# NVIDIA-AI-IOT/redtail

Hardware: AMD Instinct MI355X
Metric: stereo pairs/sec, ResNet18-2D 1257x369 (higher is better)
Workload: dtype f32

## Files before the change

redtail_amd/csrc/kernels/conv_mfma.hip.h:

```cpp
#pragma once
#include <type_traits>
#include "common.hip.h"

namespace rt {

struct ZSlice {
    int pad_y, pad_x;
    int Ho, Wo;
    int ch_row;
    unsigned tap_mask;
    int64_t y_off;
    int64_t w_off;
    int64_t r_off;
    int64_t r_off_il8;
    int64_t y_off_il8;
    int64_t r_off_il4;
};

struct ConvArgs {
    const float* x;
    float* y;
    const float* w;
    const float* bias;
    const float* resid;
    unsigned long long* dbg;
    const float* zeros;
    const ZSlice* zs;
    const int* ch_off;
    int CinPad;
    int Cout;
    int Hi, Wi;
    int x_pitch;
    int Ho, Wo;
    int pad_y, pad_x;
    int nz;
    int tiles_x;
    int act;
    int xcd_order;
    int64_t x_bstride;
    int64_t y_bstride;
    int64_t y_cstride;
    int64_t y_zstride;
    int64_t y_off;
    int y_ystride, y_xstride;
    int64_t r_cstride;
    int64_t r_bstride;
    int r_il8;
    int batch;
    int cin_real;
    int64_t x_cstride;
    const int* ch_shift;
    int w_exact;
    int z_inner;
    int nb_inner;
    int dw_seg, dw_nseg, dw_cpc, dw_ntiles;
    const float* x2;
    int x2_from;
};

#define RT_WG_TILE_NB(p, tile, zi, n, nblk)                                                         \
    int tile = blockIdx.x;                                                                          \
    if ((p).xcd_order) {                           \
        const int nwg_ = gridDim.x, q_ = nwg_ >> 3, r_ = nwg_ & 7;                                  \
        const int xcd_ = blockIdx.x & 7, idx_ = blockIdx.x >> 3;                                    \
        tile = (xcd_ < r_ ? xcd_ * (q_ + 1) : r_ * (q_ + 1) + (xcd_ - r_) * q_) + idx_;             \
    }                                                                                               \
    int nblk = blockIdx.y;                                                                          \
    if ((p).nb_inner > 0) { nblk = tile % (p).nb_inner; tile /= (p).nb_inner; }                     \
    int zi, n;                                                                                      \
    if ((p).z_inner) { zi = tile % (p).nz; tile /= (p).nz; n = blockIdx.z; }                        \
    else { zi = blockIdx.z % (p).nz; n = blockIdx.z / (p).nz; }
#define RT_WG_TILE(p, tile, zi, n) RT_WG_TILE_NB(p, tile, zi, n, nblk_unused_); (void)nblk_unused_;

#ifdef RT_KERNEL_TIMING
#define RT_TSTAMP() do { if (dbgp && tid == 0 && dbi < 16) dbgp[dbi++] = __builtin_amdgcn_s_memtime(); } while (0)
#else
#define RT_TSTAMP() do { } while (0)
#endif

#ifndef RT_ABLATE
#define RT_ABLATE 0
#endif
constexpr bool kAblGather = (RT_ABLATE & 1) != 0;
constexpr bool kAblWLoad = (RT_ABLATE & 2) != 0;
constexpr bool kAblLdsWr = (RT_ABLATE & 4) != 0;
constexpr bool kAblBarrier = (RT_ABLATE & 8) != 0;
constexpr bool kAblResid = (RT_ABLATE & 16) != 0;
constexpr bool kAblStore = (RT_ABLATE & 32) != 0;
constexpr bool kAblLdsRd = (RT_ABLATE & 64) != 0;
constexpr bool kAblXform = (RT_ABLATE & 128) != 0;
constexpr bool kAblMfma = (RT_ABLATE & 256) != 0;
__device__ __forceinline__ void wg_barrier() { if (!kAblBarrier) __syncthreads(); }

template <int N> struct VecOf;
template <> struct VecOf<2> { typedef float type __attribute__((ext_vector_type(2))); };
template <> struct VecOf<4> { typedef float type __attribute__((ext_vector_type(4))); };

template <int KH, int KW, int S, int TY, int TXW, int NBW, int CC, int NW = 4, bool WLDS = true>
struct ConvCfg {
    static constexpr int TX = 32 * TXW;
    static constexpr int NB = 32 * NBW;
    static constexpr int TAPS = KH * KW;
    static constexpr int CPG = CC / 2;
    static constexpr int PR = (TY - 1) * S + KH;
    static constexpr int PC = (TX - 1) * S + KW;
// ... 384 lines not shown
```

redtail_amd/csrc/kernels/conv_split.hip.h:

```cpp
#pragma once
#include <type_traits>
#include "common.hip.h"
#include "conv_mfma.hip.h"

namespace rt {

constexpr float kSplitScale = 2048.f;
constexpr float kSplitInv = 1.f / 2048.f;

struct S3Split {
    f16x4 hi, lo;
};
__device__ static __forceinline__ S3Split s3_split(f32x4 v) {
    S3Split s;
#ifdef HIPEMU
#pragma unroll
    for (int j = 0; j < 4; j++) {
        const _Float16 h = (_Float16)v[j];
        s.hi[j] = h;
        s.lo[j] = (_Float16)((v[j] - (float)h) * kSplitScale);
    }
#else
    unsigned h[2], l[2];
#pragma unroll
// ... 156 lines not shown
#pragma unroll
        for (int r = 0; r < 16; r++) { acc_m[r] = 0.f; acc_c[r] = 0.f; }
        const char* xb = sX[buf] + b_off;
#pragma unroll
        for (int t = 0; t < 9; t++) {
            const int r = t / 3, s = t % 3;
#pragma unroll
            for (int c = 0; c < 2; c++) {
                const char* bp = xb + (r * PC + s) * PXB + c * 32;
                const f16x8 bh = *reinterpret_cast<const f16x8*>(bp);
                const f16x8 bl = *reinterpret_cast<const f16x8*>(bp + 64);
                const f16x8 ah = __builtin_bit_cast(f16x8, sW[a_off + ((t * 2 + c) * 2 + 0) * 64]);
                const f16x8 al = __builtin_bit_cast(f16x8, sW[a_off + ((t * 2 + c) * 2 + 1) * 64]);
                acc_m = __builtin_amdgcn_mfma_f32_32x32x16_f16(ah, bh, acc_m, 0, 0, 0);
                acc_c = __builtin_amdgcn_mfma_f32_32x32x16_f16(al, bh, acc_c, 0, 0, 0);
                acc_c = __builtin_amdgcn_mfma_f32_32x32x16_f16(ah, bl, acc_c, 0, 0, 0);
            }
        }

        RT_TSTAMP();
        const buf_rsrc rs_y = make_buf(elem_ptr(p.y, (int64_t)n * p.y_bstride + p.y_off, 4));
        auto epilogue = [&](auto ACT) {
#pragma unroll
            for (int q = 0; q < 4; q++) {
                f32x4 o;
#pragma unroll
                for (int e = 0; e < 4; e++)
                    o[e] = apply_act_fast(fmaf(acc_c[4 * q + e], kSplitInv, acc_m[4 * q + e]) + (bias4[q][e] + rr[q][e]), decltype(ACT)::value);
                if constexpr (YIL) {
                    const unsigned vo = (inb && 8 * q + 4 * kg < p.Cout) ? (unsigned)((oy * p.y_ystride + ox) * 4 + 4 * kg * cs32) * 4u : kBufOOB;
                    buf_store4(o, rs_y, vo, (unsigned)(8 * q * cs32) * 4u);
                } else {
                    const unsigned vo = inb ? (unsigned)(oy * p.y_ystride + ox * p.y_xstride + 4 * kg * cs32) * 4u : kBufOOB;
#pragma unroll
                    for (int e = 0; e < 4; e++)
                        buf_store(o[e], rs_y, (8 * q + 4 * kg + e < p.Cout) ? vo : kBufOOB, (unsigned)((8 * q + e) * cs32) * 4u);
                }
            }
        };
        if (act == 1) epilogue(std::integral_constant<int, 1>{});
        else if (act == 2) epilogue(std::integral_constant<int, 2>{});
        else epilogue(std::integral_constant<int, 0>{});
        RT_TSTAMP();
    }
#ifdef RT_KERNEL_TIMING
    __builtin_amdgcn_s_waitcnt(0);
    if (dbgp && tid == 0) { dbgp[14] = __builtin_amdgcn_s_memtime(); dbgp[15] = __builtin_amdgcn_s_memrealtime() - rt0; }
#endif
}

}

namespace rt {

template <int KH, int KW, int S, int NW_ = 4>
struct S3Cfg {
    static constexpr int NW = NW_, TY = NW_, TX = 32, CC = 16, TAPS = KH * KW, NT = 64 * NW_;
    static constexpr int PR = (TY - 1) * S + KH, PC = (TX - 1) * S + KW;
    static constexpr int PCH = (PC + 1) / 2;
    static constexpr int PCL = S == 2 ? 2 * PCH : PC;
    static constexpr int NPART = NW / 4;
    static constexpr int NPIX = PR * PC, NKP = ((NPIX + NPART - 1) / NPART + 63) / 64;
    static constexpr int PXB = 80;
    static constexpr int W_SLOTS = TAPS * 2 * 2 * 32;
    static constexpr int NK_W = (W_SLOTS + NT - 1) / NT;
    static constexpr int IN_BYTES = PR * PCL * PXB, GRP_BYTES = IN_BYTES + W_SLOTS * 16;
    static constexpr int KS_MAX = NW_ != 4 ? 1 : (S == 2 ? 2 : 4);
    static constexpr int max_groups(int want) {
        int ks = want < 1 ? 1 : (want > KS_MAX ? KS_MAX : want);
        while (ks > 1 && (ks == 3 || ks * GRP_BYTES < (ks - 1) * NW * 64 * 16 * 4)) ks--;
        return ks;
    }
    static_assert(IN_BYTES % 16 == 0, "weight image alignment");
    static_assert(S == 1 || S == 2, "stride 1 or 2");
};

#ifndef RT_S3_WAVES
#define RT_S3_WAVES(S) ((S) == 2 ? 2 : 4)
#endif
template <int KH, int KW, int S, bool XIL, bool YIL, int NW = 4, typename TIN = float, typename TOUT = float>
__global__ void __launch_bounds__(64 * NW * (S3Cfg<KH, KW, S, NW>::KS_MAX)) RT_WAVES_PER_EU(RT_S3_WAVES(S)) conv_s3_kernel(ConvArgs p) {
    using Cfg = S3Cfg<KH, KW, S, NW>;
    constexpr bool XF16 = std::is_same<TIN, _Float16>::value, YF16 = std::is_same<TOUT, _Float16>::value;
    constexpr unsigned ESX = Io<TIN>::ES, ESY = Io<TOUT>::ES;
    static_assert(!XIL || !XF16, "interleaved fp16 input: conv_f16mma_kernel");
    constexpr int TY = Cfg::TY, TX = Cfg::TX, CC = Cfg::CC, TAPS = Cfg::TAPS, PC = Cfg::PC, PCL = Cfg::PCL, PXB = Cfg::PXB;
    constexpr int NKP = Cfg::NKP, NK_W = Cfg::NK_W, NT = Cfg::NT;

    constexpr int IN_BYTES = Cfg::IN_BYTES, GRP_BYTES = Cfg::GRP_BYTES;
#ifdef HIPEMU
    HIP_DYNAMIC_SHARED(char, smem)
#else
    extern __shared__ __attribute__((aligned(16))) char smem[];
#endif

    const int tid_wg = threadIdx.x;
    const int KS = Cfg::KS_MAX == 1 ? 1 : __builtin_amdgcn_readfirstlane((int)blockDim.x / NT);
    const int kgi = Cfg::KS_MAX == 1 ? 0 : __builtin_amdgcn_readfirstlane(tid_wg / NT);
    const int tid = tid_wg - kgi * NT;
    char* const sIn = smem + kgi * GRP_BYTES;
    f32x4* const sW = reinterpret_cast<f32x4*>(smem + kgi * GRP_BYTES + IN_BYTES);
#ifdef RT_KERNEL_TIMING
    unsigned long long* dbgp = (p.dbg && kgi == 0) ? p.dbg + ((size_t)(blockIdx.z * gridDim.y + blockIdx.y) * gridDim.x + blockIdx.x) * 16 : nullptr;
    int dbi = 0;
    const unsigned long long rt0 = __builtin_amdgcn_s_memrealtime();
#endif
// ... 4 lines not shown

    RT_WG_TILE_NB(p, tile, zi, n, nblk)
    const int tx0 = (tile % p.tiles_x) * TX;
    const int ty0 = (tile / p.tiles_x) * TY;
    const char* __restrict__ xb = elem_ptr(p.x, (int64_t)n * p.x_bstride, ESX);
    const int nchunks = p.CinPad / CC;
    int pad_y = p.pad_y, pad_x = p.pad_x, Ho = p.Ho, Wo = p.Wo, ch_row = zi;
    int64_t y_off = p.y_off + (int64_t)zi * p.y_zstride, w_off = 0, r_off = y_off, r_off_il8 = y_off;
    int64_t y_off_il4 = 4 * p.y_off + (int64_t)zi * p.y_zstride, r_off_il4 = y_off_il4;
    unsigned tap_mask = ~0u;
    if (p.zs) {
        const ZSlice z = p.zs[zi];
        pad_y = z.pad_y; pad_x = z.pad_x; Ho = z.Ho; Wo = z.Wo; ch_row = z.ch_row; y_off = z.y_off; w_off = z.w_off;
        r_off = z.r_off; r_off_il8 = z.r_off_il8;
        y_off_il4 = 4 * z.y_off;
        r_off_il4 = z.r_off_il4;
        tap_mask = z.tap_mask;
    }
    const int act = p.act;

    const int sg = wv & 3, spart = wv >> 2;
    const int* __restrict__ tab = p.ch_off + (int64_t)ch_row * p.CinPad + 4 * sg;
    unsigned voff[NKP];
    int lidx[NKP], xcol[NKP];
    const int* __restrict__ shtab = p.ch_shift ? p.ch_shift + (int64_t)ch_row * p.CinPad + 4 * sg : nullptr;
#pragma unroll
    for (int k = 0; k < NKP; k++) {
        const int pidx = spart * (NKP * 64) + lane + 64 * k;
        const int pr = pidx / PC, pc = pidx - pr * PC;
        const int iy = ty0 * S - pad_y + pr, ix = tx0 * S - pad_x + pc;
        const bool own = pidx < Cfg::NPIX && lane + 64 * k < NKP * 64;
        xcol[k] = ix;
        voff[k] = (own && iy >= 0 && iy < p.Hi && ix >= 0 && ix < p.Wi) ? (unsigned)(iy * p.x_pitch + ix) * (XIL ? 16u : ESX) : kBufOOB;
        const int col = S == 2 ? (pc & 1) * Cfg::PCH + (pc >> 1) : pc;
        lidx[k] = own ? (pr * PCL + col) * PXB + sg * 8 : -1;
    }
    const char* __restrict__ wsrc = reinterpret_cast<const char*>(p.w) + (w_off + ((int64_t)nblk * nchunks) * Cfg::W_SLOTS) * 16;
    const buf_rsrc rs_w = make_buf(wsrc);

    f32x4 rin[NKP];
    f32x4 rw[NK_W];
    auto prefetch = [&](int ch) {
        if constexpr (XIL) {
            const int off = tab[ch * CC];
            const int sh = shtab ? shtab[ch * CC] : 0;
            const buf_rsrc rs = make_buf(xb, off >= 0);
#pragma unroll
            for (int k = 0; k < NKP; k++) {
                const unsigned vo = sh == 0 ? voff[k] : ((voff[k] != kBufOOB && xcol[k] >= sh) ? voff[k] - (unsigned)sh * 16u : kBufOOB);
                rin[k] = buf_load4(rs, vo, (unsigned)off * 4u);
            }
        } else {
            const int sh = shtab ? shtab[ch * CC] : 0;
#pragma unroll
            for (int j = 0; j < 4; j++) {
                const int off = tab[ch * CC + j];
                const buf_rsrc rs = make_buf(xb, off >= 0);
#pragma unroll
                for (int k = 0; k < NKP; k++) {
                    const unsigned vo = sh == 0 ? voff[k] : ((voff[k] != kBufOOB && xcol[k] >= sh) ? voff[k] - (unsigned)sh * ESX : kBufOOB);
                    rin[k][j] = Io<TIN>::load(rs, vo, (unsigned)off * ESX);
                }
            }
        }
        const unsigned so = (unsigned)ch * (unsigned)(Cfg::W_SLOTS * 16);
#pragma unroll
        for (int k = 0; k < NK_W; k++) {
            const int idx = tid + NT * k;
            rw[k] = buf_load4(rs_w, idx < Cfg::W_SLOTS ? (unsigned)idx * 16u : kBufOOB, so);
        }
    };
    auto stage_to_lds = [&]() {
#pragma unroll
        for (int k = 0; k < NKP; k++) {
            if (lidx[k] < 0) continue;
            if constexpr (XF16) {
                f16x4 h;
#pragma unroll
                for (int j = 0; j < 4; j++) h[j] = (_Float16)rin[k][j];
                *reinterpret_cast<f16x4*>(sIn + lidx[k]) = h;
            } else {
                const S3Split s = s3_split(rin[k]);
                *reinterpret_cast<f16x4*>(sIn + lidx[k]) = s.hi;
                *reinterpret_cast<f16x4*>(sIn + lidx[k] + 32) = s.lo;
            }
        }
#pragma unroll
        for (int k = 0; k < NK_W; k++) {
            const int idx = tid + NT * k;
            if (idx < Cfg::W_SLOTS) sW[idx] = rw[k];
        }
    };

    const int64_t ybase = (int64_t)n * p.y_bstride + y_off;
    const int64_t rbase = (int64_t)n * p.r_bstride + r_off;
    const int cs32 = (int)p.y_cstride, rs32 = (int)p.r_cstride;
    const int oy = ty0 + wv, ox = tx0 + l31;
    const bool inb = oy < Ho && ox < Wo;
    const bool r_il = p.r_il8 != 0;
    const int cb = nblk * 32;
    f32x4 rr[4];
    if (p.resid != nullptr && kgi == 0) {
        const buf_rsrc rs_r = make_buf(elem_ptr(p.resid, r_il ? (int64_t)n * p.r_bstride + (YF16 ? r_off_il8 : r_off_il4) : rbase, ESY));
        if (r_il && YF16) {
            const unsigned vo = inb ? (unsigned)((oy * p.y_ystride + ox * p.y_xstride) * 8 + 4 * kg) * 2u : kBufOOB;
#pragma unroll
            for (int q = 0; q < 4; q++) {
                const u32x2_t u = __builtin_amdgcn_raw_buffer_load_b64(rs_r, (cb + 8 * q + 4 * kg < p.Cout) ? vo : kBufOOB, (unsigned)((cb + 8 * q) * rs32) * 2u, 0);
#pragma unroll
                for (int e = 0; e < 4; e++) rr[q][e] = (float)__builtin_bit_cast(_Float16, (unsigned short)(u[e >> 1] >> (16 * (e & 1))));
            }
        } else if (r_il) {
            const unsigned vo = inb ? (unsigned)((oy * p.y_ystride + ox * p.y_xstride) * 4 + 4 * kg * rs32) * 4u : kBufOOB;
#pragma unroll
            for (int q = 0; q < 4; q++) rr[q] = buf_load4(rs_r, (cb + 8 * q + 4 * kg < p.Cout) ? vo : kBufOOB, (unsigned)((cb + 8 * q) * rs32) * 4u);
        } else {
            const unsigned vo = inb ? (unsigned)(oy * p.y_ystride + ox * p.y_xstride + 4 * kg * rs32) * ESY : kBufOOB;
#pragma unroll
            for (int q = 0; q < 4; q++)
#pragma unroll
                for (int e = 0; e < 4; e++)
                    rr[q][e] = Io<TOUT>::load(rs_r, (cb + 8 * q + 4 * kg + e < p.Cout) ? vo : kBufOOB, (unsigned)((cb + 8 * q + e) * rs32) * ESY);
        }
    } else {
#pragma unroll
        for (int q = 0; q < 4; q++) rr[q] = f32x4{0.f, 0.f, 0.f, 0.f};
    }

    f32x16 acc_m, acc_c;
#pragma unroll
    for (int r = 0; r < 16; r++) { acc_m[r] = 0.f; acc_c[r] = 0.f; }
    const int a_off = kg * 32 + l31;
    const bool w_exact = p.w_exact != 0;
    const int b_off = (wv * S * PCL + l31) * PXB + kg * 16;
    auto compute = [&]() {
#pragma unroll
        for (int t = 0; t < TAPS; t++) {
            if (!((tap_mask >> t) & 1u)) continue;
            const int r = t / KW, s = t % KW;
            const int col = S == 2 ? (s & 1) * Cfg::PCH + (s >> 1) : s;
            const char* bp = sIn + b_off + (r * PCL + col) * PXB;
            const f16x8 bh = *reinterpret_cast<const f16x8*>(bp);
            const f16x8 ah = __builtin_bit_cast(f16x8, sW[a_off + (t * 2 + 0) * 64]);
            acc_m = __builtin_amdgcn_mfma_f32_32x32x16_f16(ah, bh, acc_m, 0, 0, 0);
            if (!w_exact) {
                const f16x8 al = __builtin_bit_cast(f16x8, sW[a_off + (t * 2 + 1) * 64]);
                acc_c = __builtin_amdgcn_mfma_f32_32x32x16_f16(al, bh, acc_c, 0, 0, 0);
            }
            if constexpr (!XF16) {
                const f16x8 bl = *reinterpret_cast<const f16x8*>(bp + 32);
                acc_c = __builtin_amdgcn_mfma_f32_32x32x16_f16(ah, bl, acc_c, 0, 0, 0);
            }
        }
    };

    if (kgi < nchunks) prefetch(kgi);
    RT_TSTAMP();
    for (int ch = kgi; ch < nchunks + kgi; ch += KS) {
        const bool mine = KS == 1 || ch < nchunks;
        if (ch != kgi) __syncthreads();
        if (mine) stage_to_lds();
        __syncthreads();
        RT_TSTAMP();
        if (ch + KS < nchunks) prefetch(ch + KS);
        if (mine) compute();
        RT_TSTAMP();
    }

#pragma unroll
    for (int r = 0; r < 16; r++) acc_m[r] = fmaf(acc_c[r], kSplitInv, acc_m[r]);
    if (KS > 1) {
        f32x4* const red = reinterpret_cast<f32x4*>(smem);
        __syncthreads();
        if (kgi > 0) {
#pragma unroll
            for (int q = 0; q < 4; q++)
                red[(((kgi - 1) * NW + wv) * 4 + q) * 64 + lane] = f32x4{acc_m[4 * q], acc_m[4 * q + 1], acc_m[4 * q + 2], acc_m[4 * q + 3]};
        }
        __syncthreads();
        if (kgi > 0) return;
        for (int g = 1; g < KS; g++)
#pragma unroll
            for (int q = 0; q < 4; q++) {
                const f32x4 v = red[(((g - 1) * NW + wv) * 4 + q) * 64 + lane];
#pragma unroll
                for (int e = 0; e < 4; e++) acc_m[4 * q + e] += v[e];
            }
    }

    const buf_rsrc rs_y = make_buf(elem_ptr(p.y, (YIL && !YF16) ? (int64_t)n * p.y_bstride + y_off_il4 : ybase, ESY));
    auto epilogue = [&](auto ACT) {
#pragma unroll
        for (int q = 0; q < 4; q++) {
            const f32x4 bv = *reinterpret_cast<const f32x4*>(p.bias + cb + 8 * q + 4 * kg);
            f32x4 o;
#pragma unroll
            for (int e = 0; e < 4; e++)
                o[e] = apply_act_fast(acc_m[4 * q + e] + (bv[e] + rr[q][e]), decltype(ACT)::value);
            if constexpr (YIL && YF16) {
                const unsigned vo = (inb && cb + 8 * q + 4 * kg < p.Cout) ? (unsigned)((oy * p.y_ystride + ox * p.y_xstride) * 8 + 4 * kg) * 2u : kBufOOB;
                u32x2_t w2;
#pragma unroll
                for (int e = 0; e < 2; e++)
                    w2[e] = (unsigned)__builtin_bit_cast(unsigned short, (_Float16)o[2 * e]) | ((unsigned)__builtin_bit_cast(unsigned short, (_Float16)o[2 * e + 1]) << 16);
                __builtin_amdgcn_raw_buffer_store_b64(w2, rs_y, vo, (unsigned)((cb + 8 * q) * cs32) * 2u, 0);
            } else if constexpr (YIL) {
                const unsigned vo = (inb && cb + 8 * q + 4 * kg < p.Cout) ? (unsigned)((oy * p.y_ystride + ox * p.y_xstride) * 4 + 4 * kg * cs32) * 4u : kBufOOB;
                buf_store4(o, rs_y, vo, (unsigned)((cb + 8 * q) * cs32) * 4u);
            } else {
                const unsigned vo = inb ? (unsigned)(oy * p.y_ystride + ox * p.y_xstride + 4 * kg * cs32) * ESY : kBufOOB;
#pragma unroll
                for (int e = 0; e < 4; e++)
                    Io<TOUT>::store(o[e], rs_y, (cb + 8 * q + 4 * kg + e < p.Cout) ? vo : kBufOOB, (unsigned)((cb + 8 * q + e) * cs32) * ESY);
            }
        }
    };
    if (act == 1) epilogue(std::integral_constant<int, 1>{});
    else if (act == 2) epilogue(std::integral_constant<int, 2>{});
    else epilogue(std::integral_constant<int, 0>{});
    RT_TSTAMP();
#ifdef RT_KERNEL_TIMING
    __builtin_amdgcn_s_waitcnt(0);
    if (dbgp && tid == 0) { dbgp[14] = __builtin_amdgcn_s_memtime(); dbgp[15] = __builtin_amdgcn_s_memrealtime() - rt0; }
#endif
}

}

namespace rt {

struct S3FirstCfg {
    static constexpr int KH = 5, KW = 5, S = 2, TY = 4, TX = 32, CMAX = 3;
    static constexpr int PR = (TY - 1) * S + KH, PC = (TX - 1) * S + KW;
    static constexpr int NPAIR = (PC + 1) / 2;
    static constexpr int RS = 208;
    static constexpr int NRUN = NPAIR / 2, NRUN_T = PR * NRUN;
    static_assert(NPAIR % 2 == 0 && NRUN_T <= 256 && (RS * 2) % 8 == 0 && NRUN * 4 * CMAX <= RS, "one gather per lane, 8-byte LDS writes");
    static constexpr int W_SLOTS = KH * 2 * 2 * 32;
};

template <bool YIL>
__global__ void __launch_bounds__(256) RT_WAVES_PER_EU(4) conv_s3_first_kernel(ConvArgs p) {
    using Cfg = S3FirstCfg;
    constexpr int KH = Cfg::KH, S = Cfg::S, TY = Cfg::TY, TX = Cfg::TX, PR = Cfg::PR, RS = Cfg::RS;

    __shared__ __attribute__((aligned(16))) _Float16 sHi[PR * RS];
    __shared__ __attribute__((aligned(16))) _Float16 sLo[PR * RS];

    const int tid = threadIdx.x;
    const int lane = tid & 63;
    const int kg = lane >> 5, l31 = lane & 31;
// ... 361 lines not shown
```

redtail_amd/csrc/rt_capi.hip:

```cpp
#include <hip/hip_runtime.h>

#include <algorithm>
#include <atomic>
#include <cmath>
#include <cstdarg>
#include <cstdio>
#include <cstdlib>
#include <cstring>
#include <string>
#include <map>
#include <mutex>
#include <vector>

#include "../../include/rt_stereo.h"
#if defined(__HIP_DEVICE_COMPILE__) && !defined(RT_BUILT_NO_SLP)
#error "rt_capi.hip must be compiled with -fno-slp-vectorize -DRT_BUILT_NO_SLP (redtail_amd/build.py: DEVICE_FLAGS)"
#endif
#include "kernels/common.hip.h"
#include "kernels/conv_mfma.hip.h"
#include "kernels/conv_wino.hip.h"
#include "kernels/deconv3d_small.hip.h"
#include "kernels/imgproc.hip.h"
#include "kernels/rectify.hip.h"
#include "kernels/speckle.hip.h"
// ... 1018 lines not shown
namespace {


struct SubConv {
    int KH = 1, KW = 1, S = 1, NBW = 1, CC = 8;
    int TY = 4, TXW = 2, NW = 4, WLDS = 1;
    int CinPad = 0, Cout = 0;
    int Hi = 0, Wi = 0, Ho = 0, Wo = 0, pad_y = 0, pad_x = 0, nz = 1;
    int x_pitch = 0;
    std::vector<rt::ZSlice> zs_host;
    int64_t y_cstride = 0, y_zstride = 0, y_off = 0;
    int64_t r_cstride = 0;
    int y_ystride = 0, y_xstride = 1;
    float* w_dev = nullptr;
    int* choff_dev = nullptr;
    int w_exact = 0;
    int* shift_dev = nullptr;
    rt::ZSlice* zs_dev = nullptr;
    int direct = 0, cin_real = 0;
    int wino = 0;
    int x_f16 = 0, y_f16 = 0;
    int f16mma = 0;
    int x_il8 = 0, y_il8 = 0, r_il8 = 0;
    int dp4 = 0;
    int f16first = 0;
    int split3 = 0;
    int rb = 0;
    int s3first = 0;
    int s3p = 0;
    int small3d = 0;
    rt::Deconv3dSmallArgs s3{};
    std::vector<float> small_w;
    void* small_il_dev = nullptr;
    int small_il_f32 = 0;
};

}

struct FoldFactor {
    rtConvPlan* pl = nullptr;
    rtConvPlan* pr = nullptr;
    float* wedge_dev = nullptr;
    int F = 0, K = 0, D = 0, H = 0, W = 0;
    int64_t a_elems = 0, c_elems = 0, t_elems = 0, e_elems = 0;
    std::mutex mu;
    std::map<rtStream, std::pair<void*, size_t>> own;
};

struct ConvKnobs {
    int xcd = 1, trace = 0;
    int rb_tiles = 0;
    int rbs_seg = 0;
    int ksplit = -1;
    int s3p_grid = 0;
    int zinner = 1;
    int nbinner = 1;
    int dw = -1;
    int dw_nseg = 0;
    int fold_u = 2;
    int f16p_walk = -1;
    int f16p_classes = 1;
    int small_walk = -1;
    int r4 = -1;
};

struct rtConvPlan {
    std::vector<SubConv> subs;
    FoldFactor* ff = nullptr;
    mutable std::once_flag env_once;
    mutable ConvKnobs opt;
    int softarg = 0;
    float* bias_dev = nullptr;
    float* zeros_dev = nullptr;
    int act = 0, has_resid = 0, dtype = RT_F32;
    int out_dims[4] = {0, 0, 0, 1};
    int64_t x_bstride = 0, y_bstride = 0;
    int64_t r_bstride = 0;
    int is2d = 0, cin = 0, hin = 0, win = 0;
    std::vector<float> w_canon;
    rtConv2dDesc desc2d{};
    int is_deconv = 0;
    int in_pitch = 0, out_pitch = 0;
    float* rb_w1_dev = nullptr;
    float* rb_bias1_dev = nullptr;
    int rb_act1 = 0, rb_cmid = 0;
    float* rbd_w1_dev = nullptr;
    float* rbd_w2_dev = nullptr;
    int x_split = 0, y_split = 0;
    float* rbh_w1_dev = nullptr;
    float* rbh_w2_dev = nullptr;
    int w_f16 = 0;
    int is_conv3d = 0, is_deconv3d = 0;
    int c3d_C = 0, c3d_cin = 0, c3d_dchw = 0, c3d_fold = 0;
    int c3d_dw = 0;
    rtConv3dDesc desc3d{};
    int in_dims3[3] = {0, 0, 0};
    int flags = 0;
};

namespace {

struct Phase1D {
    int K = 0;
    int pad = 0;
    int tap[8] = {0};
};
// ... 117 lines not shown
                    const int nb = co / 32, cc = co % 32, ch = ci / 16, h = (ci % 16) / 8, e = ci % 8;
                    packed[(size_t)base * 8 + ((((((size_t)nb * nch + ch) * taps + (u * sc.KW + v)) * 2 + h) * 32 + cc) * 8) + e] = bits;
                }
    return base;
}

int upload_zslices(SubConv& sc, const std::vector<rt::ZSlice>& zs) {
    RT_HIP(hipMalloc((void**)&sc.zs_dev, zs.size() * sizeof(rt::ZSlice)));
    RT_HIP(hipMemcpy(sc.zs_dev, zs.data(), zs.size() * sizeof(rt::ZSlice), hipMemcpyHostToDevice));
    return 0;
}

int upload_table(SubConv& sc, const std::vector<int>& table) {
    RT_HIP(hipMalloc((void**)&sc.choff_dev, table.size() * sizeof(int)));
    RT_HIP(hipMemcpy(sc.choff_dev, table.data(), table.size() * sizeof(int), hipMemcpyHostToDevice));
    return 0;
}

int upload_bias(rtConvPlan* plan, const float* bias, int n) {
    const int padded = rt::round_up(n, 64);
    std::vector<float> b(padded + 64, 0.f);
    if (bias) std::memcpy(b.data(), bias, n * sizeof(float));
    RT_HIP(hipMalloc((void**)&plan->bias_dev, b.size() * sizeof(float)));
    RT_HIP(hipMemcpy(plan->bias_dev, b.data(), b.size() * sizeof(float), hipMemcpyHostToDevice));
    plan->zeros_dev = plan->bias_dev + padded;
    return 0;
}

bool window_supported(int KH, int KW, int S) {
    if (S == 1) return (KH == 3 && KW == 3) || (KH <= 2 && KW <= 2 && KH >= 1 && KW >= 1);
    if (S == 2) return (KH == 3 && KW == 3) || (KH == 5 && KW == 5);
    return false;
}

bool dev_knobs() {
    static const bool on = [] { const char* e = getenv("RT_DEV_KNOBS"); return e && atoi(e) != 0; }();
    return on;
}
int env_int(const char* name, int dflt) {
    if (!dev_knobs()) return dflt;
    const char* e = getenv(name);
    return e ? atoi(e) : dflt;
}

#ifdef RT_EXPERIMENTAL
inline int exp_knob(const char* name, int dflt) { return env_int(name, dflt); }
#else
inline int exp_knob(const char*, int dflt) { return dflt; }
#endif
ConvKnobs read_conv_knobs() {
    ConvKnobs k;
    k.xcd = env_int("RT_CONV_XCD", k.xcd); k.trace = env_int("RT_CONV_TRACE", k.trace);
    k.rb_tiles = exp_knob("RT_RB_TILES", k.rb_tiles); k.rbs_seg = env_int("RT_RBS_SEG", k.rbs_seg); k.ksplit = env_int("RT_S3_KSPLIT", k.ksplit);
    k.s3p_grid = env_int("RT_S3P_GRID", k.s3p_grid); k.zinner = env_int("RT_Z_INNER", k.zinner); k.nbinner = env_int("RT_NB_INNER", k.nbinner);
    k.dw = env_int("RT_F16_DW", k.dw); k.dw_nseg = env_int("RT_DW_NSEG", k.dw_nseg); k.fold_u = env_int("RT_FOLD_U", k.fold_u);
    k.f16p_walk = env_int("RT_F16P_WALK", k.f16p_walk); k.f16p_classes = env_int("RT_F16P_CLASSES", k.f16p_classes);
    k.small_walk = env_int("RT_SMALL_IL_WALK", k.small_walk); k.r4 = env_int("RT_F16_R4", k.r4);
    return k;
}
thread_local int tl_exact_fp32 = 0;
int exact_fp32() { return tl_exact_fp32 || env_int("RT_CONV_EXACT_FP32", 0) != 0; }
struct ExactScope {
    int prev;
    explicit ExactScope(int flags) : prev(tl_exact_fp32) { tl_exact_fp32 = (flags & RT_CONV_EXACT_FP32) ? 1 : prev; }
    ~ExactScope() { tl_exact_fp32 = prev; }
};

void set_tile(SubConv& sc, int variant) {
    switch (variant) {
        case 0: sc.TY = 4; sc.TXW = 2; sc.NW = 4; break;
        case 4: sc.TY = 2; sc.TXW = 2; sc.NW = 4; break;
        case 9: sc.TY = 2; sc.TXW = 1; sc.NW = 2; break;
        case 8: sc.TY = 8; sc.TXW = 1; sc.NW = 8; break;
        case 10: sc.TY = 8; sc.TXW = 1; sc.NW = 4; break;
        default: sc.TY = 4; sc.TXW = 1; sc.NW = 4; break;
    }
    sc.WLDS = 1;
}

int64_t count_wgs(const SubConv& sc) {
    return rt::cdiv(sc.Ho, sc.TY) * rt::cdiv(sc.Wo, 32 * sc.TXW) * rt::cdiv(sc.Cout, 32 * sc.NBW) * sc.nz;
}

void check_direct(SubConv& sc, int cin_real) {
    const bool win = (sc.KH == sc.KW && (sc.KH == 1 || sc.KH == 2 || sc.KH == 3 || sc.KH == 5)) ||
                     (sc.KH == 1 && sc.KW == 2) || (sc.KH == 2 && sc.KW == 1);
    if (!win || (int64_t)sc.Cout * cin_real * sc.KH * sc.KW > 4096) sc.direct = 0;
}

void choose_tiling(SubConv& sc, bool allow_wino = true) {
    sc.direct = (sc.Cout <= 2 && env_int("RT_CONV_NO_DIRECT", 0) == 0) ? 1 : 0;
    sc.CC = 8;
    sc.NBW = 1;
    if (sc.KH == 5) sc.CC = 4;
    const int forced = env_int("RT_CONV_VARIANT", -1);
    set_tile(sc, forced >= 0 ? forced : 6);
    sc.wino = (allow_wino && !sc.direct && sc.KH == 3 && sc.KW == 3 && sc.S == 1 && sc.Cout >= 24 && env_int("RT_CONV_NO_WINO", 0) == 0) ? 1 : 0;
    if (sc.wino) { sc.CC = 8; sc.NBW = 1; sc.TY = exp_knob("RT_WINO_WAVES", 4); sc.TXW = 1; sc.NW = sc.TY; }
    const int nbw = env_int("RT_CONV_NBW", 0);
    if (nbw == 1 || (nbw == 2 && sc.KH != 5)) sc.NBW = nbw;
    const bool s3_win = (sc.KH == 3 && sc.KW == 3 && (sc.S == 1 || sc.S == 2)) || (sc.S == 1 && sc.KH <= 2 && sc.KW <= 2);
    sc.split3 = (!sc.direct && s3_win && !exact_fp32() && env_int("RT_NO_S3", 0) == 0) ? 1 : 0;
    if (sc.split3) {
        sc.wino = 0; sc.CC = 16; sc.NBW = 1; sc.TY = 4; sc.TXW = 1; sc.NW = 4;
        if (sc.KH == 3 && sc.KW == 3 && sc.S == 1 && exp_knob("RT_S3_ROWS", 4) == 8) sc.TY = sc.NW = 8;
    }
// ... 1514 lines not shown
            const int64_t waves = (int64_t)groups * rowpairs * batch;
            int nseg = (int)std::min<int64_t>(std::max<int64_t>(1, rt::cdiv((int64_t)8 * device_cus(), waves)), std::max(1, a.Mz / 8));
            const int seg_len = (int)rt::cdiv(a.Mz, nseg);
            nseg = (int)rt::cdiv(a.Mz, seg_len);
            RT_REQUIRE(rowpairs <= 65535, "rt_conv_enqueue: grid limit exceeded");
            dim3 gw((unsigned)(rt::cdiv(groups, 4) * nseg), (unsigned)rowpairs, (unsigned)batch);
            if (plan->opt.trace) fprintf(stderr, "[rt] deconv3d_s2_ilw<0> grid %u x %u x %u segments %d x %d\n", gw.x, gw.y, gw.z, nseg, seg_len);
            hipLaunchKernelGGL(rt::deconv3d_s2_ilw_kernel<0>, gw, dim3(256), 0, S(L.s), a, seg_len, nseg);
        } else {
            dim3 g2((unsigned)(rt::cdiv(groups, 4 * rt::kSmallIlIters) * a.Mz), (unsigned)rowpairs, (unsigned)batch);
            if (plan->opt.trace) fprintf(stderr, "[rt] deconv3d_s2_il grid %u x %u x %u\n", g2.x, g2.y, g2.z);
            hipLaunchKernelGGL(rt::deconv3d_s2_il_kernel, g2, dim3(256), 0, S(L.s), a);
        }
    } else if (sc.small3d == 1 && !sc.x_f16 && sc.x_il8) {
        RT_REQUIRE(sc.small_il_dev && sc.small_il_f32, "rt_conv_enqueue: interleaved fp32 input without its weight operands (rt_conv_plan_set_layouts)");
        a.w = static_cast<const float*>(sc.small_il_dev);
        const int groups = (int)rt::cdiv((a.Wx + 1) / 2, 16);
        RT_REQUIRE(batch <= 65535, "rt_conv_enqueue: grid limit exceeded");
        dim3 g2((unsigned)(rt::cdiv(groups, 4 * rt::kSmallIlIters) * a.Mz), (unsigned)rt::cdiv((a.Hx + 1) / 2, 2), (unsigned)batch);
        if (plan->opt.trace) fprintf(stderr, "[rt] deconv3d_s2_il4 grid %u x %u x %u\n", g2.x, g2.y, g2.z);
        hipLaunchKernelGGL(rt::deconv3d_s2_il4_kernel, g2, dim3(256), 0, S(L.s), a);
    } else if (sc.small3d == 1 && sc.x_f16) {
        if (a.C == 1) hipLaunchKernelGGL((rt::deconv3d_s2_small_kernel<1, true, _Float16, float>), grid, dim3(256), 0, S(L.s), a);
        else hipLaunchKernelGGL((rt::deconv3d_s2_small_kernel<2, true, _Float16, float>), grid, dim3(256), 0, S(L.s), a);
    } else if (sc.small3d == 2) {
        if (a.C == 1) hipLaunchKernelGGL((rt::deconv3d_s2_small_kernel<1, false>), grid, dim3(256), 0, S(L.s), a);
        else hipLaunchKernelGGL((rt::deconv3d_s2_small_kernel<2, false>), grid, dim3(256), 0, S(L.s), a);
    } else {
        if (a.C == 1) hipLaunchKernelGGL((rt::deconv3d_s2_small_kernel<1, true>), grid, dim3(256), 0, S(L.s), a);
        else hipLaunchKernelGGL((rt::deconv3d_s2_small_kernel<2, true>), grid, dim3(256), 0, S(L.s), a);
    }
    RT_LAUNCH_CHECK("deconv3d_s2_small_kernel");
    return 0;
}

rt::ConvArgs conv_args(const Launch& L, const SubConv& sc) {
    const rtConvPlan* plan = L.plan;
    rt::ConvArgs a;
    a.z_inner = 0; a.nb_inner = 0;
    a.x = static_cast<const float*>(L.x);
    a.x2 = static_cast<const float*>(L.x2); a.x2_from = L.x2_from;
    a.y = static_cast<float*>(L.y);
    a.w = sc.w_dev;
    a.bias = plan->bias_dev;
    a.zeros = plan->zeros_dev;
    a.dbg = nullptr;
#ifdef RT_KERNEL_TIMING
    if (const char* e = getenv("RT_DBG_PTR")) a.dbg = (unsigned long long*)strtoull(e, nullptr, 0);
#endif
    a.resid = plan->has_resid ? static_cast<const float*>(L.residual) : nullptr;
    a.ch_off = sc.choff_dev;
    a.ch_shift = sc.shift_dev;
    a.w_exact = plan->w_f16;
    a.zs = sc.zs_dev;
    a.CinPad = sc.CinPad; a.Cout = sc.Cout;
    a.Hi = sc.Hi; a.Wi = sc.Wi; a.Ho = sc.Ho; a.Wo = sc.Wo;
    a.x_pitch = sc.x_pitch ? sc.x_pitch : sc.Wi;
    a.pad_y = sc.pad_y; a.pad_x = sc.pad_x; a.nz = sc.nz;
    a.tiles_x = (int)rt::cdiv(sc.Wo, 32 * sc.TXW);
    a.act = plan->act;
    a.xcd_order = plan->opt.xcd;
    a.x_bstride = plan->x_bstride; a.y_bstride = plan->y_bstride;
    a.y_cstride = sc.y_cstride; a.y_zstride = sc.y_zstride; a.y_off = sc.y_off;
    if (plan->is_conv3d && !plan->c3d_dchw && sc.y_il8) a.y_zstride = 8 * sc.y_zstride;
    a.y_ystride = sc.y_ystride; a.y_xstride = sc.y_xstride;
    a.r_cstride = sc.r_cstride ? sc.r_cstride : sc.y_cstride;
    a.r_bstride = plan->r_bstride ? plan->r_bstride : plan->y_bstride;
    a.r_il8 = sc.r_il8;
    a.batch = L.batch; a.cin_real = sc.cin_real; a.x_cstride = (int64_t)sc.Hi * a.x_pitch;
    return a;
}

int enqueue_deconv_s3p(const Launch& L, const SubConv& sc, rt::ConvArgs& a) {
    a.tiles_x = (int)rt::cdiv(sc.Wi, 32);
    const int tiles = a.tiles_x * (int)rt::cdiv(sc.Hi, 4), nblk = (int)rt::cdiv(sc.Cout, 32);
    RT_REQUIRE(!sc.x_il8 && !sc.x_f16 && !sc.y_f16, "rt_conv_enqueue: the fp32 four-phase transposed kernel takes a planar fp32 input and writes fp32");
    RT_REQUIRE((int64_t)L.batch * sc.nz <= 65535, "rt_conv_enqueue: grid limit exceeded");
    RT_REQUIRE(sc.y_cstride * (int64_t)sc.Cout < (1ll << 29), "rt_conv_enqueue: output sample exceeds 2 GB (32-bit buffer offsets)");
    dim3 g((unsigned)tiles, (unsigned)nblk, (unsigned)(L.batch * sc.nz));
    if (L.plan->opt.trace) fprintf(stderr, "[rt] deconv_s3p<%d> r%d grid %u x %u x %u\n", sc.y_il8 ? 1 : 0, sc.r_il8, g.x, g.y, g.z);
    if (sc.y_il8) hipLaunchKernelGGL(rt::deconv_s3p_kernel<true>, g, dim3(256), 0, S(L.s), a);
    else hipLaunchKernelGGL(rt::deconv_s3p_kernel<false>, g, dim3(256), 0, S(L.s), a);
    RT_LAUNCH_CHECK("deconv_s3p_kernel");
    return 0;
}

int enqueue_deconv_f16p(const Launch& L, const SubConv& sc, rt::ConvArgs& a, bool& took_next) {
    const rtConvPlan* plan = L.plan;
    const int batch = L.batch;
    a.tiles_x = (int)rt::cdiv(sc.Wi, 32);
    const int tiles = a.tiles_x * (int)rt::cdiv(sc.Hi, 4), nblk = (int)rt::cdiv(sc.Cout, 32);
    RT_REQUIRE(sc.x_il8 && sc.y_il8 && sc.x_f16 && sc.y_f16, "rt_conv_enqueue: the four-phase transposed kernel takes interleaved fp16 tensors");
    a.z_inner = plan->opt.zinner != 0 ? 1 : 0;
    RT_REQUIRE(batch <= 65535 && (int64_t)batch * sc.nz <= 65535, "rt_conv_enqueue: grid limit exceeded");
    dim3 g = a.z_inner ? dim3((unsigned)(tiles * sc.nz), (unsigned)nblk, (unsigned)batch) : dim3((unsigned)tiles, (unsigned)nblk, (unsigned)(batch * sc.nz));
    if (plan->opt.f16p_walk != 0 && (!plan->has_resid || sc.r_il8)) {
        rt::DeconvWalkB wb{};
        const SubConv* sb = (&sc == &plan->subs[0] && plan->subs.size() == 2) ? &plan->subs[1] : nullptr;
        if (sb && plan->opt.f16p_classes != 0 && sb->dp4 && sb->f16mma && sb->x_il8 && sb->y_il8 && sb->x_f16 && sb->y_f16 && sb->r_il8 == sc.r_il8 &&
            sb->Hi == sc.Hi && sb->Wi == sc.Wi && sb->Ho == sc.Ho && sb->Wo == sc.Wo && sb->Cout == sc.Cout && sb->x_pitch == sc.x_pitch &&
            sb->y_cstride == sc.y_cstride && sb->y_ystride == sc.y_ystride && sb->r_cstride == sc.r_cstride) {
            wb.w = static_cast<const float*>(sb->w_dev); wb.zs = sb->zs_dev; wb.ch_off = sb->choff_dev; wb.CinPad = sb->CinPad; wb.nz = sb->nz;
            took_next = true;
        }
        const int nzw = std::max(sc.nz, wb.zs ? wb.nz : 0);
        const double per_m = wb.zs ? (double)(sc.CinPad + wb.CinPad) / sc.CinPad : 1.0;
// ... 611 lines not shown
```

Measured before the change: 2762.

## Software-pipeline S3 split-conv MFMA loop and defer bias/residual loads to last chunk

Restructures the split-fp16 conv inner loop so each tap's LDS operand loads for the next tap are issued before the current tap's MFMAs. Sched barriers and opaque uniform tap masks pin this interleaving. The bias and residual reads move into the final chunk iteration, overlapping them with the last compute instead of issuing them up front. The input gather is specialised on whether a channel shift is present, and the weight-load offsets are simplified to a per-thread base plus a constant. The risks are higher register pressure from the double-buffered operands, and rigid scheduling that may block compiler optimisations.

```diff
diff --git a/redtail_amd/csrc/kernels/conv_mfma.hip.h b/redtail_amd/csrc/kernels/conv_mfma.hip.h
--- a/redtail_amd/csrc/kernels/conv_mfma.hip.h
+++ b/redtail_amd/csrc/kernels/conv_mfma.hip.h
@@ -51,6 +51,7 @@
     int64_t x_cstride;
     const int* ch_shift;
     int w_exact;
+    int s3_general;
     int z_inner;
     int nb_inner;
     int dw_seg, dw_nseg, dw_cpc, dw_ntiles;
diff --git a/redtail_amd/csrc/kernels/conv_split.hip.h b/redtail_amd/csrc/kernels/conv_split.hip.h
--- a/redtail_amd/csrc/kernels/conv_split.hip.h
+++ b/redtail_amd/csrc/kernels/conv_split.hip.h
@@ -232,6 +232,13 @@
 }
 
 namespace rt {
+
+__device__ static __forceinline__ unsigned s3_opaque(unsigned v) {
+#ifndef HIPEMU
+    asm volatile("" : "+s"(v));
+#endif
+    return v;
+}
 
 template <int KH, int KW, int S, int NW_ = 4>
 struct S3Cfg {
@@ -342,22 +349,27 @@
             }
         } else {
             const int sh = shtab ? shtab[ch * CC] : 0;
-#pragma unroll
-            for (int j = 0; j < 4; j++) {
-                const int off = tab[ch * CC + j];
-                const buf_rsrc rs = make_buf(xb, off >= 0);
-#pragma unroll
-                for (int k = 0; k < NKP; k++) {
-                    const unsigned vo = sh == 0 ? voff[k] : ((voff[k] != kBufOOB && xcol[k] >= sh) ? voff[k] - (unsigned)sh * ESX : kBufOOB);
-                    rin[k][j] = Io<TIN>::load(rs, vo, (unsigned)off * ESX);
+            auto gather = [&](auto shifted) {
+#pragma unroll
+                for (int j = 0; j < 4; j++) {
+                    const int off = tab[ch * CC + j];
+                    const buf_rsrc rs = make_buf(xb, off >= 0);
+#pragma unroll
+                    for (int k = 0; k < NKP; k++) {
+                        unsigned vo = voff[k];
+                        if constexpr (decltype(shifted)::value) vo = (voff[k] != kBufOOB && xcol[k] >= sh) ? voff[k] - (unsigned)sh * ESX : kBufOOB;
+                        rin[k][j] = Io<TIN>::load(rs, vo, (unsigned)off * ESX);
+                    }
                 }
-            }
+            };
+            if (sh == 0) gather(std::false_type{});
+            else gather(std::true_type{});
         }
         const unsigned so = (unsigned)ch * (unsigned)(Cfg::W_SLOTS * 16);
 #pragma unroll
         for (int k = 0; k < NK_W; k++) {
-            const int idx = tid + NT * k;
-            rw[k] = buf_load4(rs_w, idx < Cfg::W_SLOTS ? (unsigned)idx * 16u : kBufOOB, so);
+            const bool in = NT * (k + 1) <= Cfg::W_SLOTS || tid + NT * k < Cfg::W_SLOTS;
+            rw[k] = buf_load4(rs_w, in ? (unsigned)tid * 16u : kBufOOB, so + (unsigned)(NT * k * 16));
         }
     };
     auto stage_to_lds = [&]() {
@@ -389,33 +401,37 @@
     const bool inb = oy < Ho && ox < Wo;
     const bool r_il = p.r_il8 != 0;
     const int cb = nblk * 32;
-    f32x4 rr[4];
-    if (p.resid != nullptr && kgi == 0) {
-        const buf_rsrc rs_r = make_buf(elem_ptr(p.resid, r_il ? (int64_t)n * p.r_bstride + (YF16 ? r_off_il8 : r_off_il4) : rbase, ESY));
-        if (r_il && YF16) {
-            const unsigned vo = inb ? (unsigned)((oy * p.y_ystride + ox * p.y_xstride) * 8 + 4 * kg) * 2u : kBufOOB;
-#pragma unroll
-            for (int q = 0; q < 4; q++) {
-                const u32x2_t u = __builtin_amdgcn_raw_buffer_load_b64(rs_r, (cb + 8 * q + 4 * kg < p.Cout) ? vo : kBufOOB, (unsigned)((cb + 8 * q) * rs32) * 2u, 0);
-#pragma unroll
-                for (int e = 0; e < 4; e++) rr[q][e] = (float)__builtin_bit_cast(_Float16, (unsigned short)(u[e >> 1] >> (16 * (e & 1))));
-            }
-        } else if (r_il) {
-            const unsigned vo = inb ? (unsigned)((oy * p.y_ystride + ox * p.y_xstride) * 4 + 4 * kg * rs32) * 4u : kBufOOB;
-#pragma unroll
-            for (int q = 0; q < 4; q++) rr[q] = buf_load4(rs_r, (cb + 8 * q + 4 * kg < p.Cout) ? vo : kBufOOB, (unsigned)((cb + 8 * q) * rs32) * 4u);
+    f32x4 rr[4], bv[4];
+    auto request_tail = [&]() {
+#pragma unroll
+        for (int q = 0; q < 4; q++) bv[q] = *reinterpret_cast<const f32x4*>(p.bias + cb + 8 * q + 4 * kg);
+        if (p.resid != nullptr) {
+            const buf_rsrc rs_r = make_buf(elem_ptr(p.resid, r_il ? (int64_t)n * p.r_bstride + (YF16 ? r_off_il8 : r_off_il4) : rbase, ESY));
+            if (r_il && YF16) {
+                const unsigned vo = inb ? (unsigned)((oy * p.y_ystride + ox * p.y_xstride) * 8 + 4 * kg) * 2u : kBufOOB;
+#pragma unroll
+                for (int q = 0; q < 4; q++) {
+                    const u32x2_t u = __builtin_amdgcn_raw_buffer_load_b64(rs_r, (cb + 8 * q + 4 * kg < p.Cout) ? vo : kBufOOB, (unsigned)((cb + 8 * q) * rs32) * 2u, 0);
+#pragma unroll
+                    for (int e = 0; e < 4; e++) rr[q][e] = (float)__builtin_bit_cast(_Float16, (unsigned short)(u[e >> 1] >> (16 * (e & 1))));
+                }
+            } else if (r_il) {
+                const unsigned vo = inb ? (unsigned)((oy * p.y_ystride + ox * p.y_xstride) * 4 + 4 * kg * rs32) * 4u : kBufOOB;
+#pragma unroll
+                for (int q = 0; q < 4; q++) rr[q] = buf_load4(rs_r, (cb + 8 * q + 4 * kg < p.Cout) ? vo : kBufOOB, (unsigned)((cb + 8 * q) * rs32) * 4u);
+            } else {
+                const unsigned vo = inb ? (unsigned)(oy * p.y_ystride + ox * p.y_xstride + 4 * kg * rs32) * ESY : kBufOOB;
+#pragma unroll
+                for (int q = 0; q < 4; q++)
+#pragma unroll
+                    for (int e = 0; e < 4; e++)
+                        rr[q][e] = Io<TOUT>::load(rs_r, (cb + 8 * q + 4 * kg + e < p.Cout) ? vo : kBufOOB, (unsigned)((cb + 8 * q + e) * rs32) * ESY);
+            }
         } else {
-            const unsigned vo = inb ? (unsigned)(oy * p.y_ystride + ox * p.y_xstride + 4 * kg * rs32) * ESY : kBufOOB;
-#pragma unroll
-            for (int q = 0; q < 4; q++)
-#pragma unroll
-                for (int e = 0; e < 4; e++)
-                    rr[q][e] = Io<TOUT>::load(rs_r, (cb + 8 * q + 4 * kg + e < p.Cout) ? vo : kBufOOB, (unsigned)((cb + 8 * q + e) * rs32) * ESY);
-        }
-    } else {
-#pragma unroll
-        for (int q = 0; q < 4; q++) rr[q] = f32x4{0.f, 0.f, 0.f, 0.f};
-    }
+#pragma unroll
+            for (int q = 0; q < 4; q++) rr[q] = f32x4{0.f, 0.f, 0.f, 0.f};
+        }
+    };
 
     f32x16 acc_m, acc_c;
 #pragma unroll
@@ -423,36 +439,65 @@
     const int a_off = kg * 32 + l31;
     const bool w_exact = p.w_exact != 0;
     const int b_off = (wv * S * PCL + l31) * PXB + kg * 16;
+    auto b_ptr = [&](int t) {
+        const int r = t / KW, s = t % KW;
+        const int col = S == 2 ? (s & 1) * Cfg::PCH + (s >> 1) : s;
+        return sIn + b_off + (r * PCL + col) * PXB;
+    };
+    auto op_bh = [&](int t) { return *reinterpret_cast<const f16x8*>(b_ptr(t)); };
+    auto op_bl = [&](int t) { return *reinterpret_cast<const f16x8*>(b_ptr(t) + 32); };
+    auto op_ah = [&](int t) { return __builtin_bit_cast(f16x8, sW[a_off + (t * 2 + 0) * 64]); };
+    auto op_al = [&](int t) { return __builtin_bit_cast(f16x8, sW[a_off + (t * 2 + 1) * 64]); };
+    const unsigned taps_all = (1u << TAPS) - 1u;
+    const unsigned live_m = __builtin_amdgcn_readfirstlane((tap_mask & taps_all) | (p.s3_general != 0 ? 0x80000000u : 0u));
+    const unsigned live_c = __builtin_amdgcn_readfirstlane(w_exact ? 0u : (tap_mask & taps_all));
     auto compute = [&]() {
+        f16x8 al = op_al(0), bh = op_bh(0), ah = op_ah(0), bl = bh;
+        if constexpr (!XF16) bl = op_bl(0);
 #pragma unroll
         for (int t = 0; t < TAPS; t++) {
-            if (!((tap_mask >> t) & 1u)) continue;
-            const int r = t / KW, s = t % KW;
-            const int col = S == 2 ? (s & 1) * Cfg::PCH + (s >> 1) : s;
-            const char* bp = sIn + b_off + (r * PCL + col) * PXB;
-            const f16x8 bh = *reinterpret_cast<const f16x8*>(bp);
-            const f16x8 ah = __builtin_bit_cast(f16x8, sW[a_off + (t * 2 + 0) * 64]);
-            acc_m = __builtin_amdgcn_mfma_f32_32x32x16_f16(ah, bh, acc_m, 0, 0, 0);
-            if (!w_exact) {
-                const f16x8 al = __builtin_bit_cast(f16x8, sW[a_off + (t * 2 + 1) * 64]);
-                acc_c = __builtin_amdgcn_mfma_f32_32x32x16_f16(al, bh, acc_c, 0, 0, 0);
-            }
+            const bool more = t + 1 < TAPS;
+            const unsigned lm = s3_opaque(live_m), lc = s3_opaque(live_c);
+            f16x8 aln = al, bhn = bh, ahn = ah, bln = bl;
+            if (more) { aln = op_al(t + 1); bhn = op_bh(t + 1); }
+            __builtin_amdgcn_sched_barrier(0);
+            if (lm >> 31) __builtin_amdgcn_s_waitcnt(0xC07F);
+            if ((lc >> t) & 1u) acc_c = __builtin_amdgcn_mfma_f32_32x32x16_f16(al, bh, acc_c, 0, 0, 0);
+            __builtin_amdgcn_sched_barrier(0);
+            if (more) ahn = op_ah(t + 1);
+            __builtin_amdgcn_sched_barrier(0);
+            if ((lm >> t) & 1u) acc_m = __builtin_amdgcn_mfma_f32_32x32x16_f16(ah, bh, acc_m, 0, 0, 0);
+            __builtin_amdgcn_sched_barrier(0);
             if constexpr (!XF16) {
-                const f16x8 bl = *reinterpret_cast<const f16x8*>(bp + 32);
-                acc_c = __builtin_amdgcn_mfma_f32_32x32x16_f16(ah, bl, acc_c, 0, 0, 0);
-            }
-        }
-    };
-
+                if (more) bln = op_bl(t + 1);
+                __builtin_amdgcn_sched_barrier(0);
+                if ((lm >> t) & 1u) acc_c = __builtin_amdgcn_mfma_f32_32x32x16_f16(ah, bl, acc_c, 0, 0, 0);
+                __builtin_amdgcn_sched_barrier(0);
+            }
+            al = aln; bh = bhn; ah = ahn; bl = bln;
+        }
+    };
+
+    const int rounds = (nchunks + KS - 1) / KS;
+    int ch = kgi;
     if (kgi < nchunks) prefetch(kgi);
     RT_TSTAMP();
-    for (int ch = kgi; ch < nchunks + kgi; ch += KS) {
-        const bool mine = KS == 1 || ch < nchunks;
-        if (ch != kgi) __syncthreads();
+    for (int rd = 0; rd + 1 < rounds; rd++, ch += KS) {
+        if (rd != 0) __syncthreads();
+        stage_to_lds();
+        __syncthreads();
+        RT_TSTAMP();
+        if (ch + KS < nchunks) prefetch(ch + KS);
+        compute();
+        RT_TSTAMP();
+    }
+    {
+        const bool mine = ch < nchunks;
+        if (rounds > 1) __syncthreads();
         if (mine) stage_to_lds();
         __syncthreads();
         RT_TSTAMP();
-        if (ch + KS < nchunks) prefetch(ch + KS);
+        if (kgi == 0) request_tail();
         if (mine) compute();
         RT_TSTAMP();
     }
@@ -482,11 +527,10 @@
     auto epilogue = [&](auto ACT) {
 #pragma unroll
         for (int q = 0; q < 4; q++) {
-            const f32x4 bv = *reinterpret_cast<const f32x4*>(p.bias + cb + 8 * q + 4 * kg);
             f32x4 o;
 #pragma unroll
             for (int e = 0; e < 4; e++)
-                o[e] = apply_act_fast(acc_m[4 * q + e] + (bv[e] + rr[q][e]), decltype(ACT)::value);
+                o[e] = apply_act_fast(acc_m[4 * q + e] + (bv[q][e] + rr[q][e]), decltype(ACT)::value);
             if constexpr (YIL && YF16) {
                 const unsigned vo = (inb && cb + 8 * q + 4 * kg < p.Cout) ? (unsigned)((oy * p.y_ystride + ox * p.y_xstride) * 8 + 4 * kg) * 2u : kBufOOB;
                 u32x2_t w2;
diff --git a/redtail_amd/csrc/rt_capi.hip b/redtail_amd/csrc/rt_capi.hip
--- a/redtail_amd/csrc/rt_capi.hip
+++ b/redtail_amd/csrc/rt_capi.hip
@@ -1094,6 +1094,7 @@
     int rb_tiles = 0;
     int rbs_seg = 0;
     int ksplit = -1;
+    int s3_general = 0;
     int s3p_grid = 0;
     int zinner = 1;
     int nbinner = 1;
@@ -1317,6 +1318,7 @@
     ConvKnobs k;
     k.xcd = env_int("RT_CONV_XCD", k.xcd); k.trace = env_int("RT_CONV_TRACE", k.trace);
     k.rb_tiles = exp_knob("RT_RB_TILES", k.rb_tiles); k.rbs_seg = env_int("RT_RBS_SEG", k.rbs_seg); k.ksplit = env_int("RT_S3_KSPLIT", k.ksplit);
+    k.s3_general = env_int("RT_S3_GENERAL", k.s3_general);
     k.s3p_grid = env_int("RT_S3P_GRID", k.s3p_grid); k.zinner = env_int("RT_Z_INNER", k.zinner); k.nbinner = env_int("RT_NB_INNER", k.nbinner);
     k.dw = env_int("RT_F16_DW", k.dw); k.dw_nseg = env_int("RT_DW_NSEG", k.dw_nseg); k.fold_u = env_int("RT_FOLD_U", k.fold_u);
     k.f16p_walk = env_int("RT_F16P_WALK", k.f16p_walk); k.f16p_classes = env_int("RT_F16P_CLASSES", k.f16p_classes);
@@ -2937,6 +2939,7 @@
     a.ch_off = sc.choff_dev;
     a.ch_shift = sc.shift_dev;
     a.w_exact = plan->w_f16;
+    a.s3_general = plan->opt.s3_general != 0;
     a.zs = sc.zs_dev;
     a.CinPad = sc.CinPad; a.Cout = sc.Cout;
     a.Hi = sc.Hi; a.Wi = sc.Wi; a.Ho = sc.Ho; a.Wo = sc.Wo;
```

Result: no change. 2757 (-0.2%).
